# awslabs/flowgger

Measured on AMD Instinct MI355X. Metric: log lines/sec (RFC5424, 256B avg) at 1/2/4/8 MI355X; achieved HBM GB/s, higher is better.
Workload: dtype u8; 1 GPU; BASELINE configs[1]: RFC5424 no structured data, 100000000 lines/GPU @ 254 B avg (1000000-line tile x100 resident in HBM), 1% invalid lines; lines_per_gpu=100000000, bytes_per_gpu=25376525600, parallelism=lines sharded 1-way, no data-path collective, ok_lines_per_tile=990000

## Files before the change

flowgger_amd/csrc/fg_gelf.hip:

```cpp
#include "fg_fused.hpp"
#include "fg_numparse.hpp"
#include "fg_gelf2.hpp"

namespace fg {

using namespace gelf2;

enum : uint32_t { J_OK = 0, J_SYNTAX = 1, J_CTRL = 2 };
constexpr uint32_t V_NESTED = 6;
constexpr uint32_t kMaxDepth = 512;
constexpr uint32_t kMaxStored = 32;

struct Member {
    uint32_t key_b, key_e, key_esc;
    uint32_t kind;
    uint32_t v_b, v_e, v_esc;
    uint64_t bits;
    uint32_t end;
};

template <class R>
struct Gelf {
    R& rd;
    uint32_t len;
// ... 400 lines not shown
                    --j;
                }
                keypos[j] = pi;
            }
        }
        for (uint32_t i = 0; i < n; ++i) {
            Member m;
            g.member(keypos[i], &m);
            if (i + 1 < n) {
                uint32_t ne, nesc;
                g.scan_string(keypos[i + 1] + 1, &ne, &nesc);
                if (g.key_cmp(m.key_b, m.key_e, m.key_esc, keypos[i + 1] + 1, ne, nesc) == 0) continue;
            }
            uint32_t st = gelf_dispatch<EMIT>(g, m, r, t, slot, &cnt);
            if (st != G_OK) {
                r.status = st;
                return;
            }
        }
    } else {
        bool have_prev = false;
        Member prev;
        for (;;) {
            bool have_best = false;
            Member best;
            uint32_t p = g.skip_ws(0) + 1;
            for (uint32_t k = 0; k < n; ++k) {
                p = g.skip_ws(p);
                if (k) p = g.skip_ws(p + 1);
                Member m;
                g.member(p, &m);
                p = m.end;
                if (have_prev && g.key_cmp(m.key_b, m.key_e, m.key_esc, prev.key_b, prev.key_e, prev.key_esc) <= 0) continue;
                if (!have_best || g.key_cmp(m.key_b, m.key_e, m.key_esc, best.key_b, best.key_e, best.key_esc) <= 0) {
                    best = m;
                    have_best = true;
                }
            }
            if (!have_best) break;
            uint32_t st = gelf_dispatch<EMIT>(g, best, r, t, slot, &cnt);
            if (st != G_OK) {
                r.status = st;
                return;
            }
            prev = best;
            have_prev = true;
        }
    }
    if (!EMIT) r.n_ent = cnt;
}

template <class R>
__device__ __forceinline__ void gelf_line(R& rd, uint32_t len, uint32_t* keypos, uint32_t* stack, GRow& r, const DevTables& t) {
    Gelf<R> g{rd, len, false, stack};
    bool is_object = false;
    uint32_t e = gelf_validate(g, keypos, r, &is_object);
    if (e == J_CTRL) {
        g.retry = true;
        r = GRow();
        e = gelf_validate(g, keypos, r, &is_object);
        if (e == J_OK) r.flags |= FG_F_GELF_RETRY;
    }
    if (e != J_OK) {
        r.status = G_JSON;
        return;
    }
    if (!is_object) {
        r.status = G_EMPTY;
        return;
    }
    gelf_sorted_dispatch<false>(g, keypos, r, t, 0);
    if (r.status != G_OK) return;
    if (!r.have_ts) r.flags |= FG_F_TS_NOW;
    if (!r.have_host) r.status = G_NOHOST;
}

constexpr uint32_t kGelfLines = 64;
constexpr uint32_t kPending = 0xFCu;

inline uint32_t gelf_extra_lds(uint32_t tile, uint32_t lines) { return gelf2::extra_bytes(tile, lines); }

struct GelfFormat {
    static constexpr uint32_t kClasses = gelf2::kClasses;
    static __device__ __forceinline__ void classify_store(const uint4& q, uint16_t* bm16, uint32_t chunk, uint32_t stride, uint32_t term4) {
        uint32_t m[gelf2::kClasses + 1];
        gelf2::classify(q.x, q.y, q.z, q.w, m, term4);
        gelf2::store_classes(m, bm16, chunk, stride);
    }
    uint8_t* extra;
    uint32_t tile_cap, lines;
    unsigned long long* pacc;

    __device__ __forceinline__ RowOut decode(const GroupCtx& c, const DevTables& t) const {
        const uint32_t lane = threadIdx.x;
        const uint32_t len = (uint32_t)(c.o1 - c.o0);
        const bool in_tile = (c.o1 - c.a0) <= (uint64_t)c.span;
        const uint32_t base = (uint32_t)(c.o0 - c.a0);
        gelf2::Lds L = gelf2::carve(c.smem, c.bm16, tile_cap, extra, lines);
        L.ent_state = c.ent_state;
        L.alloc_chunk = t.alloc_chunk;
        const bool tile_lane = c.valid && in_tile && lane < lines && !(c.ablate & 4u);
        const gelf2::LineOut f = c.phase ? gelf2::decode_tile<true>(L, c.span, tile_lane, base, len, t, pacc)
                                         : gelf2::decode_tile<false>(L, c.span, tile_lane, base, len, t);
        RowOut o;
        const fg_span none{0, FG_NONE};
        const bool ok = f.handled && f.status == G_OK;
        o.meta = f.handled ? (f.status | (0xFFu << 8) | ((ok ? f.severity : 0xFFu) << 16) | ((ok ? f.flags : 0u) << 24)) : kPending;
        if (t.pending && c.valid && !f.handled) gstore(t.pending, 0, t.epoch);
        o.ts = (ok && f.have_ts) ? f.ts : 0.0;
        o.span[S_HOST] = ok ? fg_span{f.host_off, f.host_len} : none;
        o.span[S_APP] = none;
        o.span[S_PROC] = none;
        o.span[S_MSGID] = none;
        o.span[S_MSG] = ok ? fg_span{f.msg_off, f.msg_len} : none;
        o.span[S_FULL] = ok ? fg_span{f.full_off, f.full_len} : none;
        o.first = f.handled ? f.first : 0u;
        o.count = f.handled ? f.n_ent : 0u;
        return o;
    }
};

template <int NB, bool PROF, int MINW = 4, uint32_t TILE = 0, uint32_t LINES = 0>
__global__ __launch_bounds__(kWave, MINW) void k_gelf(const uint8_t* __restrict__ bytes, const uint64_t* __restrict__ offsets,
                                                  uint64_t n, DevTables t, uint32_t tile_cap_, uint32_t L_, uint64_t groups,
                                                  unsigned long long* prof, uint64_t* stash_base, FrameArgs fr) {
    const uint32_t tile_cap = TILE ? TILE : tile_cap_, L = LINES ? LINES : L_;
    extern __shared__ __attribute__((aligned(16))) uint8_t smem[];
    __shared__ unsigned long long pacc[PROF ? 10 : 1];
    GelfFormat fmt{smem + tile_cap + 64u + (tile_cap / 16u + 16u) * 2u * GelfFormat::kClasses, tile_cap, L, pacc};
    if (PROF && threadIdx.x < 10) pacc[threadIdx.x] = 0ull;
    {
        const gelf2::Lds lds = gelf2::carve(smem, reinterpret_cast<uint16_t*>(smem + tile_cap + 64u), tile_cap, fmt.extra, L);
        gelf2::init_lds(lds);
        gelf2::clear_dirty(lds, tile_cap);
    }
    __shared__ DevTables t_lds;
    if (threadIdx.x == 0) t_lds = t;
    __syncthreads();
    persistent_loop<NB, PROF>(bytes, offsets, n, t_lds, tile_cap, L, groups, prof, stash_base, fmt, fr);
    if (PROF) {
        __syncthreads();
        if (threadIdx.x < 10) atomicAdd(&prof[6 + threadIdx.x], pacc[threadIdx.x]);
    }
}

template <int NB, int MINW = 4, uint32_t TILE = 0, uint32_t LINES = 0>
__global__ __launch_bounds__(kWave, MINW) void k_gelf_fused(const uint8_t* __restrict__ bytes, DevTables t, uint32_t tile_cap_, uint32_t L_,
                                                         FusedArgs fa, uint32_t strip) {
    const uint32_t tile_cap = TILE ? TILE : tile_cap_, L = LINES ? LINES : L_;
    extern __shared__ __attribute__((aligned(16))) uint8_t smem[];
    GelfFormat fmt{smem + tile_cap + 64u + (tile_cap / 16u + 16u) * 2u * GelfFormat::kClasses, tile_cap, L, nullptr};
    {
        const gelf2::Lds lds = gelf2::carve(smem, reinterpret_cast<uint16_t*>(smem + tile_cap + 64u), tile_cap, fmt.extra, L);
        gelf2::init_lds(lds);
        gelf2::clear_dirty(lds, tile_cap);
    }
    __shared__ DevTables t_lds;
    __shared__ FusedArgs fa_lds;
    if (threadIdx.x == 0) {
        t_lds = t;
        fa_lds = fa;
    }
    __syncthreads();
    fused_loop<NB>(bytes, t_lds, tile_cap, L, fmt, fa_lds, strip, nullptr);
}

// ... 205 lines not shown
```

flowgger_amd/csrc/fg_pipeline.hpp:

```cpp
#pragma once
#include "fg_device.hpp"
#include "fg_plan_policy.hpp"
#include "fg_sparse_need.hpp"
#include "fg_wave.hpp"

namespace fg {

using u32x4 = unsigned int __attribute__((ext_vector_type(4)));

__device__ __forceinline__ uint32_t eq_flags(uint32_t x, uint32_t pat) {
    uint32_t s = ((x & 0x7F7F7F7Fu) ^ pat) + 0x7F7F7F7Fu;
    return ~(s | x) & 0x80808080u;
}
__device__ __forceinline__ uint32_t range_flags(uint32_t x) {
    uint32_t l = x & 0x7F7F7F7Fu;
    uint32_t ge33 = l + 0x5F5F5F5Fu;
    uint32_t le126 = l + 0x01010101u;
    return ge33 & ~le126 & ~x & 0x80808080u;
}
__device__ __forceinline__ uint32_t ctrl_flags(uint32_t x) {
    uint32_t ge32 = (x & 0x7F7F7F7Fu) + 0x60606060u;
    return ~(ge32 | x) & 0x80808080u;
}
__device__ __forceinline__ uint32_t gather16(uint32_t f0, uint32_t f1, uint32_t f2, uint32_t f3) {
// ... 149 lines not shown
    uint32_t span;
    bool valid;
    uint64_t li;
    uint64_t* stash;
    uint32_t ablate;
    uint32_t* ent_state;
    unsigned long long* phase;
    uint32_t tbase = 0;
    uint32_t tlen = 0;
    uint32_t last2 = 0;
    uint32_t tile_cap = 0;
};

template <uint32_t WORDS, class Unpack>
__device__ __forceinline__ bool stash_to_table(const GroupCtx& c, const DevTables& t, const EntAlloc& a, uint32_t n_ent, bool mine,
                                               Unpack un) {
    const uint32_t lane = threadIdx.x;
    const uint32_t cap = (c.span / 18u) & ~3u;
    if (a.total == 0u || a.total > cap || a.s.overflow || c.stash == nullptr || __any(n_ent != 0u && !mine)) return false;
    uint64_t* s_name = reinterpret_cast<uint64_t*>(const_cast<uint8_t*>(c.smem));
    uint64_t* s_val = s_name + cap;
    uint16_t* s_tf = reinterpret_cast<uint16_t*>(s_val + cap);
    __syncthreads();
    for (uint32_t k0 = 0; k0 < n_ent; k0 += 4u) {
        uint64_t w0[4], w1[4];
#pragma unroll
        for (uint32_t j = 0; j < 4u; ++j) {
            const uint32_t k = k0 + j < n_ent ? k0 + j : n_ent - 1u;
            w0[j] = c.stash[(k * WORDS) * kWave + lane];
            w1[j] = WORDS > 1u ? c.stash[(k * WORDS + 1u) * kWave + lane] : 0ull;
        }
#pragma unroll
        for (uint32_t j = 0; j < 4u; ++j) {
            if (k0 + j < n_ent) {
                uint64_t name, val;
                uint32_t tf;
                un(w0[j], w1[j], &name, &val, &tf);
                const uint32_t idx = a.ex + k0 + j;
                s_name[idx] = name;
                s_val[idx] = val;
                s_tf[idx] = (uint16_t)tf;
            }
        }
    }
    __syncthreads();
    for (uint32_t idx = lane; idx < a.total; idx += kWave) {
        const uint32_t slot = a.s.at(idx);
        const uint64_t name = s_name[idx];
        const uint32_t tf = s_tf[idx];
        t.ent_name[slot] = fg_span{(uint32_t)name, (uint32_t)(name >> 32)};
        t.ent_val[slot] = s_val[idx];
        t.ent_type[slot] = (uint8_t)(tf & 0xFFu);
        t.ent_flags[slot] = (uint8_t)(tf >> 8);
    }
    return true;
}


struct FrameArgs {
    uint32_t strip;
    const uint8_t* line_bad;
    uint32_t* ticket = nullptr;
    uint32_t ticket_base = 0;
    uint32_t taper0 = kNoTaper, taper1 = kNoTaper, taper2 = kNoTaper;
};

#define FG_STREAM_AUX 2
__device__ __forceinline__ uint4 stream_load(const uint4* p) {
    typedef uint32_t nt4 __attribute__((ext_vector_type(4)));
    const nt4 v = __builtin_nontemporal_load(reinterpret_cast<const nt4*>(p));
    return make_uint4(v.x, v.y, v.z, v.w);
}

template <class F, class = void>
struct tail_batch { static constexpr int value = 4; };
template <class F>
struct tail_batch<F, decltype((void)F::kTailBatch)> { static constexpr int value = F::kTailBatch; };

template <class F, class = void>
struct defer_row_store { static constexpr bool value = true; };
template <class F>
struct defer_row_store<F, decltype((void)F::kDeferRowStore)> { static constexpr bool value = F::kDeferRowStore; };

constexpr uint32_t kHeadCap = 1024;
template <class F, class = void>
struct head_cap { static constexpr uint32_t value = kHeadCap; };
template <class F>
struct head_cap<F, decltype((void)F::kHeadBytes)> { static constexpr uint32_t value = F::kHeadBytes; };

constexpr uint32_t kSparseHandful = 4;

template <int NB, bool PROF, class F, bool HEAD = false, uint32_t SPARSE = 0>
__device__ __forceinline__ void persistent_loop(const uint8_t* __restrict__ bytes, const uint64_t* __restrict__ offsets,
                                                uint64_t n, const DevTables& t, uint32_t tile_cap, uint32_t L, uint64_t chunk_lines,
                                                unsigned long long* prof, uint64_t* stash_base, F& fmt, FrameArgs fr) {
    static_assert(!HEAD || F::kClasses <= 1, "HEAD staging classifies one stage-A byte class at most");
    static_assert(SPARSE == 0 || (!HEAD && F::kClasses == 0), "the sparse window builds its need bitmap where a stage-A class bitmap would lie");
    static_assert(SPARSE % 16u == 0 && SPARSE <= 112u, "a line's run of chunks (at most (H + 4 + 14) / 16 + 1) must fit two bitmap words at any shift");
    const uint64_t kChunkLines = chunk_lines;
    extern __shared__ __attribute__((aligned(16))) uint8_t smem[];
    uint16_t* bm16 = reinterpret_cast<uint16_t*>(smem + tile_cap + 64u);
    const uint32_t bm_stride = tile_cap / 16u + 16u;
    uint4* dst = reinterpret_cast<uint4*>(smem);
    const uint32_t lane = threadIdx.x;
    const uint64_t G = gridDim.x;
    uint64_t* stash = stash_base ? stash_base + (uint64_t)blockIdx.x * (kStashEntries * kStashWords * kWave) : nullptr;

    const bool dyn = fr.ticket != nullptr;
    uint32_t tk_raw = 0;
    bool tk_pending = false;
    auto draw_ticket = [&]() {
        if (lane == 0u) tk_raw = __hip_atomic_fetch_add(fr.ticket, 1u, __ATOMIC_RELAXED, __HIP_MEMORY_SCOPE_AGENT);
        tk_pending = true;
    };
    uint64_t chunk = blockIdx.x;
    uint64_t p, hi_line;
    chunk_range(chunk, kChunkLines, fr.taper0, fr.taper1, fr.taper2, n, &p, &hi_line);
    if (dyn && p < n) draw_ticket();

    auto load_offsets = [&](uint64_t q, uint64_t* o0, uint64_t* o1) {
        const uint64_t li = q + lane;
        const bool in = lane < L && li < hi_line;
        *o0 = offsets[in ? li : hi_line];
        *o1 = offsets[in ? li + 1 : hi_line];
    };
    auto geometry = [&](uint64_t q, uint64_t o0, uint64_t o1, uint32_t* nl, uint64_t* a0, uint32_t* span) {
        const uint64_t left = hi_line - q;
        const uint32_t avail = left < (uint64_t)L ? (uint32_t)left : L;
        const uint32_t lo_l = (uint32_t)__builtin_amdgcn_readfirstlane((int)(uint32_t)o0);
        const uint32_t lo_h = (uint32_t)__builtin_amdgcn_readfirstlane((int)(uint32_t)(o0 >> 32));
        const uint64_t lo = (uint64_t)lo_l | ((uint64_t)lo_h << 32);
        *a0 = lo & ~15ull;
        const unsigned long long fit = __ballot(lane < avail && (o1 - *a0) <= (uint64_t)tile_cap);
        uint32_t cnt = fit == ~0ull ? 64u : (uint32_t)__builtin_ctzll(~fit);
        if (cnt == 0u) cnt = 1u;
        *nl = cnt;
        const uint32_t last = cnt - 1u;
        const uint32_t hi_l = (uint32_t)__builtin_amdgcn_readlane((int)(uint32_t)o1, (int)last);
        const uint32_t hi_h = (uint32_t)__builtin_amdgcn_readlane((int)(uint32_t)(o1 >> 32), (int)last);
        const uint64_t hi = (uint64_t)hi_l | ((uint64_t)hi_h << 32);
        const uint64_t want = hi - *a0;
        *span = want > tile_cap ? tile_cap : (uint32_t)((want + 15ull) & ~15ull);
    };
    auto load_window = [&](uint64_t a0, uint32_t span, u32x4* v) {
        __amdgpu_buffer_rsrc_t rsrc =
            __builtin_amdgcn_make_buffer_rsrc(const_cast<uint8_t*>(bytes + a0), (short)0, (int)span, 0x00020000);
#pragma unroll
        for (int k = 0; k < NB; ++k) v[k] = __builtin_amdgcn_raw_buffer_load_b128(rsrc, (int)(lane * 16u + k * 1024u), 0, FG_STREAM_AUX);
    };
    const uint32_t sparse_tail = fr.strip != FG_FRAME_NONE ? kSparseTailFramed : kSparseTailPlain;
    auto sparse_offsets = [&](uint64_t a0_, uint32_t span_, uint32_t nl_, uint64_t lo0, uint64_t lo1, bool dense, uint32_t* vo) {
        uint32_t* skip = reinterpret_cast<uint32_t*>(bm16);
        const uint32_t nchunk_ = span_ >> 4;
        const uint32_t nwin = nchunk_ < (uint32_t)NB * kWave ? nchunk_ : (uint32_t)NB * kWave;
        const uint32_t nword = 2u * NB + 2u < tile_cap / 32u + 8u ? 2u * NB + 2u : tile_cap / 32u + 8u;
        if (lane < nword) {
            const uint32_t c = lane * 32u;
            skip[lane] = !dense || c >= nchunk_ ? ~0u : nchunk_ - c >= 32u ? 0u : ~0u << (nchunk_ - c);
        }
        __syncthreads();
        if (!dense) {
            auto mark = [&](const NeedRange& r, bool on) {
                const bool go = on && r.n != 0u && r.c0 < nwin;
                const uint64_t m = go ? ((1ull << r.n) - 1ull) << (r.c0 & 31u) : 0ull;
                const uint32_t w = go ? r.c0 >> 5 : 0u;
                __hip_atomic_fetch_and(skip + w, ~(uint32_t)m, __ATOMIC_RELAXED, __HIP_MEMORY_SCOPE_WORKGROUP);
                __hip_atomic_fetch_and(skip + w + 1u, ~(uint32_t)(m >> 32), __ATOMIC_RELAXED, __HIP_MEMORY_SCOPE_WORKGROUP);
            };
            const uint32_t t0 = (uint32_t)lo0 - (uint32_t)a0_, t1 = (uint32_t)lo1 - (uint32_t)a0_;
            mark(need_head(t0, t1 - t0, SPARSE, sparse_tail, lane == 0u), lane < nl_);
            if (lane + 1u == nl_) mark(need_tail(t1, sparse_tail), true);
            __syncthreads();
        }
        const uint32_t half = lane >> 5, bit = lane & 31u, off = lane * 16u;
#pragma unroll
        for (int k = 0; k < NB; ++k) vo[k] = ((skip[2 * k + (int)half] >> bit) << 31) | off;
    };
    auto load_window_sparse = [&](uint64_t a0_, uint32_t span_, const uint32_t* vo, u32x4* v) {
        __amdgpu_buffer_rsrc_t rsrc =
            __builtin_amdgcn_make_buffer_rsrc(const_cast<uint8_t*>(bytes + a0_), (short)0, (int)span_, 0x00020000);
#pragma unroll
        for (int k = 0; k < NB; ++k) v[k] = __builtin_amdgcn_raw_buffer_load_b128(rsrc, (int)vo[k], k * 1024, FG_STREAM_AUX);
    };
    auto geometry_head = [&](uint64_t q, uint64_t o0, uint64_t o1, uint32_t* nl, uint32_t* span, uint32_t* st_out, uint32_t* tb_out) {
        const uint64_t left = hi_line - q;
        const uint32_t avail = left < (uint64_t)L ? (uint32_t)left : L;
        const uint64_t want = (o1 - o0) + (o0 & 15ull);
        uint32_t st = want >= head_cap<F>::value ? head_cap<F>::value : (uint32_t)((want + 15ull) & ~15ull);
        if (lane >= avail) st = 0u;
        uint32_t total;
        const uint32_t tb = wv::excl_sum(st, &total);
        const unsigned long long fit = __ballot(lane < avail && tb + st <= tile_cap);
        uint32_t cnt = fit == ~0ull ? 64u : (uint32_t)__builtin_ctzll(~fit);
        if (cnt == 0u) cnt = 1u;
        *nl = cnt;
        const uint32_t last = cnt - 1u;
        *span = (uint32_t)__builtin_amdgcn_readlane((int)tb, (int)last) + (uint32_t)__builtin_amdgcn_readlane((int)st, (int)last);
        *st_out = lane < cnt ? st : 0u;
        *tb_out = tb;
    };
    auto load_window_head = [&](uint64_t o0, uint32_t st, u32x4* v) {
#pragma unroll
        for (int k = 0; k < NB; ++k) {
            const uint32_t lo = (uint32_t)__builtin_amdgcn_readlane((int)(uint32_t)o0, k);
            const uint32_t hi = (uint32_t)__builtin_amdgcn_readlane((int)(uint32_t)(o0 >> 32), k);
            const uint32_t sk = (uint32_t)__builtin_amdgcn_readlane((int)st, k);
            const uint64_t b = ((uint64_t)lo | ((uint64_t)hi << 32)) & ~15ull;
            __amdgpu_buffer_rsrc_t rsrc = __builtin_amdgcn_make_buffer_rsrc(const_cast<uint8_t*>(bytes + b), (short)0, (int)sk, 0x00020000);
            v[k] = __builtin_amdgcn_raw_buffer_load_b128(rsrc, (int)(lane * 16u), 0, FG_STREAM_AUX);
        }
    };
    auto load_last2 = [&](uint64_t o0, uint64_t o1) -> uint32_t {
        const uint64_t len = o1 - o0;
        uint32_t r = 0;
        if (len >= 1u) r = bytes[o1 - 1u];
        if (len >= 2u) r |= (uint32_t)bytes[o1 - 2u] << 8;
        return r;
    };

    uint32_t* ent_state = reinterpret_cast<uint32_t*>(smem + tile_cap + 56u);
    if (lane < 2u) ent_state[lane] = 0u;
    if (p >= hi_line) return;
    uint64_t o0, o1, a0 = 0;
    uint32_t span, nl, st = 0, tb = 0, last2 = 0;
    load_offsets(p, &o0, &o1);
    u32x4 v[NB];
    if constexpr (HEAD) {
        geometry_head(p, o0, o1, &nl, &span, &st, &tb);
        load_window_head(o0, st, v);
        last2 = load_last2(o0, o1);
    } else if constexpr (SPARSE != 0) {
        geometry(p, o0, o1, &nl, &a0, &span);
        uint32_t vo[NB];
        sparse_offsets(a0, span, nl, o0, o1, false, vo);
        load_window_sparse(a0, span, vo, v);
    } else {
        geometry(p, o0, o1, &nl, &a0, &span);
        load_window(a0, span, v);
    }
    bool dense = false, dense_next = false, dense_then = false;
    RowOut pend{};
    uint64_t pend_li = 0;
    bool pend_valid = false;
    uint64_t acc0 = 0, acc1 = 0, acc2 = 0, acc3 = 0, iters = 0, tm0 = 0, tm1 = 0, tm2 = 0, tm3 = 0;
    const uint32_t ablate = PROF ? (uint32_t)prof[5] : 0u;
    const uint32_t term4 = fr.strip == FG_FRAME_LINE ? 0x0A0A0A0Au : fr.strip == FG_FRAME_NUL ? 0u : wv::kNoTerm;

    for (;;) {
        uint64_t pn = p + nl;
        if (pn >= hi_line) {
            if (dyn) {
                if (!tk_pending) draw_ticket();
                const uint32_t tk = (uint32_t)__builtin_amdgcn_readfirstlane((int)tk_raw);
                chunk = (uint64_t)(uint32_t)(tk - fr.ticket_base) + G;
                tk_pending = false;
                chunk_range(chunk, kChunkLines, fr.taper0, fr.taper1, fr.taper2, n, &pn, &hi_line);
                if (pn < n) draw_ticket();
            } else {
                chunk += G;
                chunk_range(chunk, kChunkLines, kNoTaper, kNoTaper, kNoTaper, n, &pn, &hi_line);
            }
        }
        const bool more = pn < n;
        uint64_t no0 = 0, no1 = 0;
        if (more) load_offsets(pn, &no0, &no1);
        if (PROF) {
            tm0 = __builtin_amdgcn_s_memtime();
            __builtin_amdgcn_s_waitcnt(0x0F70);
            tm1 = __builtin_amdgcn_s_memtime();
        }
        FG_MARK(A);
        const uint32_t nchunk = span >> 4;
        const uint32_t nrow = HEAD ? nl : (nchunk + kWave - 1u) / kWave;
        if constexpr (HEAD) {
#pragma unroll
            for (int k = 0; k < NB; ++k) {
                if ((uint32_t)k < nl) {
                    const uint32_t tk = (uint32_t)__builtin_amdgcn_readlane((int)tb, k), sk = (uint32_t)__builtin_amdgcn_readlane((int)st, k);
                    if (lane * 16u < sk) {
                        const uint4 q = make_uint4(v[k][0], v[k][1], v[k][2], v[k][3]);
                        dst[(tk >> 4) + lane] = q;
                        if constexpr (F::kClasses != 0) F::classify_store(q, bm16, (tk >> 4) + lane, bm_stride, term4);
                    }
                }
            }
            constexpr uint32_t HB = tail_batch<F>::value >= 8 ? 8u : 4u;
            for (uint32_t r0 = NB; r0 < nl; r0 += HB) {
                uint4 w[HB];
                uint32_t tk[HB], sk[HB];
#pragma unroll
                for (uint32_t j = 0; j < HB; ++j) {
                    const uint32_t r = r0 + j < nl ? r0 + j : nl - 1u;
                    const uint32_t lo = (uint32_t)__builtin_amdgcn_readlane((int)(uint32_t)o0, (int)r);
                    const uint32_t hi = (uint32_t)__builtin_amdgcn_readlane((int)(uint32_t)(o0 >> 32), (int)r);
                    tk[j] = (uint32_t)__builtin_amdgcn_readlane((int)tb, (int)r);
                    sk[j] = (uint32_t)__builtin_amdgcn_readlane((int)st, (int)r);
                    const uint64_t b = ((uint64_t)lo | ((uint64_t)hi << 32)) & ~15ull;
                    __amdgpu_buffer_rsrc_t rsrc = __builtin_amdgcn_make_buffer_rsrc(const_cast<uint8_t*>(bytes + b), (short)0, (int)sk[j], 0x00020000);
                    const u32x4 x = __builtin_amdgcn_raw_buffer_load_b128(rsrc, (int)(lane * 16u), 0, FG_STREAM_AUX);
                    w[j] = make_uint4(x[0], x[1], x[2], x[3]);
                }
#pragma unroll
                for (uint32_t j = 0; j < HB; ++j)
                    if (lane * 16u < sk[j]) {
                        dst[(tk[j] >> 4) + lane] = w[j];
                        if constexpr (F::kClasses != 0) F::classify_store(w[j], bm16, (tk[j] >> 4) + lane, bm_stride, term4);
                    }
            }
        } else {
#pragma unroll
        for (int k = 0; k < NB; ++k) {
            if ((uint32_t)k < nrow) {
                uint32_t idx = k * kWave + lane;
                uint4 q = make_uint4(v[k][0], v[k][1], v[k][2], v[k][3]);
                dst[idx] = q;
                F::classify_store(q, bm16, idx, bm_stride, idx < nchunk ? term4 : wv::kPastSpan);
            }
        }
        }
        if (!HEAD && nrow > (uint32_t)NB) {
            const uint4* __restrict__ src = reinterpret_cast<const uint4*>(bytes + a0);
            const uint32_t last = nchunk - 1u;
            constexpr int TB = tail_batch<F>::value;
            for (uint32_t c0 = NB * kWave; c0 < nchunk; c0 += kWave * TB) {
                uint4 w[TB];
#pragma unroll
                for (int k = 0; k < TB; ++k) {
                    const uint32_t idx = c0 + k * kWave + lane;
                    w[k] = stream_load(src + (idx < last ? idx : last));
                }
#pragma unroll
                for (int k = 0; k < TB; ++k) {
                    if (k == 0 || c0 + k * kWave < nchunk) {
                        const uint32_t idx = c0 + k * kWave + lane, ci = idx < last ? idx : last;
                        dst[ci] = w[k];
                        F::classify_store(w[k], bm16, ci, bm_stride, term4);
                    }
                }
            }
            if constexpr (SPARSE != 0) __builtin_amdgcn_s_waitcnt(0x0F70);
        }
        __builtin_amdgcn_sched_barrier(0);
        FG_MARK(S);
        if (PROF) {
            __builtin_amdgcn_s_waitcnt(0xC07F);
            tm2 = __builtin_amdgcn_s_memtime();
        }
        uint64_t pa0 = 0;
        uint32_t pspan = 0, pnl = 0, pst = 0, ptb = 0, plast2 = 0;
        if (more) {
            if constexpr (HEAD) geometry_head(pn, no0, no1, &pnl, &pspan, &pst, &ptb);
            else geometry(pn, no0, no1, &pnl, &pa0, &pspan);
        }
        uint32_t pvo[SPARSE != 0 ? NB : 1];
        if constexpr (SPARSE != 0) {
            dense_next = dense_then;
            if (more) sparse_offsets(pa0, pspan, pnl, no0, no1, dense_next, pvo);
        }
        FG_MARK(ST);
        if (pend_valid && !(ablate & 1u)) store_row(t, pend_li, pend);
        FG_MARK(W0);
        if (more) {
            if constexpr (HEAD) {
                load_window_head(no0, pst, v);
                plast2 = load_last2(no0, no1);
            } else if constexpr (SPARSE != 0) {
                load_window_sparse(pa0, pspan, pvo, v);
            } else {
                load_window(pa0, pspan, v);
            }
        }
        __builtin_amdgcn_sched_barrier(0);
        FG_MARK(W1);
        FG_MARK(B);
        if (PROF) tm3 = __builtin_amdgcn_s_memtime();
        __syncthreads();
        if (!(ablate & 2u)) {
            const uint64_t li = p + lane;
            const bool valid = lane < nl;
            uint64_t e1 = o1;
            uint32_t l2 = last2;
            if (fr.strip != FG_FRAME_NONE) {
                uint32_t b1 = last2 & 0xFFu, b2 = (last2 >> 8) & 0xFFu;
                if constexpr (!HEAD) {
                    const uint64_t len = o1 - o0;
                    const bool over = nl == 1u && __builtin_amdgcn_readfirstlane((int)((o1 - a0) > (uint64_t)span)) != 0;
                    if (over) {
                        FG_RARE_BEGIN();
                        if (valid && len >= 1u) b1 = bytes[o1 - 1u];
                        if (valid && len >= 2u) b2 = bytes[o1 - 2u];
                        FG_RARE_END();
                    } else if (valid) {
                        const uint32_t q = (uint32_t)(o1 - a0);
                        if (len >= 1u) b1 = smem[q - 1u];
                        if (len >= 2u) b2 = smem[q - 2u];
                    }
                }
                if (valid && e1 > o0) {
                    if (fr.strip == FG_FRAME_LINE) {
                        if (b1 == '\n') {
                            --e1;
                            if (e1 > o0 && b2 == '\r') --e1;
                        }
                    } else if (b1 == 0u) {
                        --e1;
                    }
                    if (HEAD && e1 != o1) {
                        l2 = 0u;
                        if (e1 - o0 >= 1u) l2 = bytes[e1 - 1];
                        if (e1 - o0 >= 2u) l2 |= (uint32_t)bytes[e1 - 2] << 8;
                    }
                }
            }
            GroupCtx c{bytes, smem, bm16, o0, e1, a0, span, valid, li, (ablate & 8u) ? nullptr : stash, ablate, ent_state, PROF ? prof + 6 : nullptr};
            c.tile_cap = tile_cap;
            if constexpr (HEAD) {
                const uint32_t al = (uint32_t)(o0 & 15ull), len = (uint32_t)(e1 - o0);
                c.tbase = tb + al;
                c.tlen = st == 0u ? 0u : (st - al < len ? st - al : len);
                c.last2 = l2;
            }
            if constexpr (SPARSE != 0) {
                const uint32_t len = (uint32_t)(e1 - o0);
                c.tbase = (uint32_t)(o0 - a0);
                c.tlen = dense || len < SPARSE ? len : SPARSE;
                c.last2 = 0u;
                if (valid && e1 > o0 && (o1 - a0) <= (uint64_t)span) {
                    const uint32_t q = (uint32_t)(e1 - a0);
                    c.last2 = smem[q - 1u];
                    if (len >= 2u) c.last2 |= (uint32_t)smem[q - 2u] << 8;
                }
            }
            pend = fmt.decode(c, t);
            if constexpr (SPARSE != 0) {
                const uint32_t nh = (uint32_t)__popcll(__ballot(valid && pend.handed));
                dense_then = dense ? nh != 0u : nh > kSparseHandful;
            }
            if (fr.line_bad && valid && fr.line_bad[li]) {
                pend.meta = FG_ST_BAD_UTF8 | (0xFFu << 8) | (0xFFu << 16);
                pend.ts = 0.0;
#pragma unroll
                for (int k = 0; k < 6; ++k) pend.span[k] = fg_span{0, FG_NONE};
                pend.count = 0;
            }
            pend_li = li;
            pend_valid = valid;
            if (!defer_row_store<F>::value) {
                if (pend_valid && !(ablate & 1u)) store_row(t, pend_li, pend);
                pend_valid = false;
            }
        }
        if (PROF) {
            __builtin_amdgcn_sched_barrier(0);
            __builtin_amdgcn_s_waitcnt(0xC07F);
            uint64_t tm4 = __builtin_amdgcn_s_memtime();
            acc0 += tm1 - tm0;
            acc1 += tm2 - tm1;
            acc2 += tm3 - tm2;
            acc3 += tm4 - tm3;
            iters += 1;
        }
        FG_MARK(Z);
        if (!more) break;
        __syncthreads();
        p = pn;
        nl = pnl;
        o0 = no0;
        o1 = no1;
        a0 = pa0;
        span = pspan;
        if constexpr (SPARSE != 0) dense = dense_next;
        if constexpr (HEAD) {
            st = pst;
            tb = ptb;
            last2 = plast2;
        }
    }
    if (pend_valid && !(ablate & 1u)) store_row(t, pend_li, pend);
    if (PROF && lane == 0) {
        atomicAdd(&prof[0], (unsigned long long)acc0);
        atomicAdd(&prof[1], (unsigned long long)acc1);
        atomicAdd(&prof[2], (unsigned long long)acc2);
        atomicAdd(&prof[3], (unsigned long long)acc3);
        atomicAdd(&prof[4], (unsigned long long)iters);
    }
}

}

#include <cstdio>
#include <cstdlib>

#include "fg_cus.hpp"

namespace fg {
constexpr int kComputeBoundWindow = 2;

inline void take_tickets(FrameArgs* fr, TicketSlot* tk, const LaunchPlan& p) {
    if (!tk || !tk->d_word || !tk->h_val || p.chunks + p.blocks >= 0xFFFFFFFFull || p.blocks > p.chunks) return;
    if (!p.tickets) return;
    fr->ticket = tk->d_word;
    fr->ticket_base = *tk->h_val;
    fr->taper0 = p.taper[0], fr->taper1 = p.taper[1], fr->taper2 = p.taper[2];
    *tk->h_val += (uint32_t)p.chunks;
}

template <class K>
inline int plan_launch(K kernel, uint64_t n, uint64_t avg_len, uint32_t extra_lds, uint32_t max_tile, uint32_t stash_blocks, LaunchPlan* p,
                       const fg_launch_opts& lo, const PlanFormat& pf = PlanFormat()) {
    static_cast<LaunchGeometry&>(*p) = launch_geometry(n, avg_len, extra_lds, max_tile, lo, pf);
    const int cus = device_cus();
    if (cus < 1) return -1;
    int per_cu = 0;
    if (hipOccupancyMaxActiveBlocksPerMultiprocessor(&per_cu, kernel, kWave, p->lds) != hipSuccess || per_cu < 1) per_cu = 1;
    if (lo.waves_per_cu > 0 && per_cu > (int)lo.waves_per_cu) per_cu = (int)lo.waves_per_cu;
    uint64_t blocks = (uint64_t)per_cu * (uint64_t)cus;
    if (blocks > p->groups) blocks = p->groups;
    if (stash_blocks && blocks > stash_blocks) blocks = stash_blocks;
    const ChunkPlan cp = plan_chunks(n, blocks, p->L, p->g, p->full, pf.ticket_from, lo, pf.taper);
    p->chunk = cp.chunk;
    p->chunks = cp.chunks;
    p->tickets = cp.tickets;
    for (int j = 0; j < 3; ++j) p->taper[j] = cp.taper[j];
    p->blocks = cp.blocks;
    return 0;
}

#if defined(FG_PROF_BUILD)
inline bool prof_requested() { return getenv("FG_PROF") != nullptr; }
#define FG_PROF_TWIN(...) (__VA_ARGS__)
#else
constexpr bool prof_requested() { return false; }
#define FG_PROF_TWIN(...) nullptr
#endif
struct ProfRun {
    unsigned long long* d = nullptr;
    unsigned long long h[16] = {0, 0, 0, 0, 0, 0, 0, 0, 0, 0, 0, 0, 0, 0, 0, 0};
    bool begin(hipStream_t stream) {
#if defined(FG_PROF_BUILD)
        if (const char* e = getenv("FG_ABLATE")) h[5] = (unsigned long long)atoi(e);
#endif
        if (hipMalloc((void**)&d, sizeof(h)) != hipSuccess) return false;
        (void)hipMemcpyAsync(d, h, sizeof(h), hipMemcpyHostToDevice, stream);
        return true;
    }
    void end(hipStream_t stream, const char* name, const LaunchPlan& p) {
        (void)hipStreamSynchronize(stream);
        (void)hipMemcpy(h, d, sizeof(h), hipMemcpyDeviceToHost);
        (void)hipFree(d);
        const double it = h[4] ? (double)h[4] : 1.0;
        fprintf(stderr,
// ... 55 lines not shown
```

flowgger_amd/csrc/fg_rfc5424.hip:

```cpp
#include <cstdio>
#include <cstdlib>

#include "fg_fused.hpp"
#include "fg_sd2.hpp"
#include "fg_tsfast.hpp"

namespace fg {

enum : uint32_t {
    E_OK = 0,
    E_BOM = 1,
    E_BRACKETS = 2,
    E_INVPRI = 3,
    E_NOVER = 4,
    E_BADVER = 5,
    E_NOTS = 6,
    E_BADTS = 7,
    E_NOHOST = 8,
    E_NOAPP = 9,
    E_NOPROC = 10,
    E_NOMSGID = 11,
    E_NODATA = 12,
    E_NOMSG = 13,
    E_MALFORMED = 14,
// ... 826 lines not shown
                sd_walk<true>(rd, r.data0, len, &msg_at, &cnt, t, first);
            } else {
                FG_RARE_BEGIN();
                GlobalReader rd(reinterpret_cast<const uint32_t*>(bytes), o0);
                sd_walk<true>(rd, r.data0, len, &msg_at, &cnt, t, first);
                FG_RARE_END();
            }
        }
    }

    tick(8);
    RowOut o;
    const bool ok = r.status == E_OK;
    o.meta = r.status | (r.facility << 8) | (r.severity << 16) | (r.flags << 24);
    o.ts = ok ? r.ts : 0.0;
#pragma unroll
    for (int k = 0; k < 6; ++k) o.span[k] = ok ? fg_span{r.off[k], r.len[k]} : fg_span{0, FG_NONE};
    o.first = first;
    o.count = r.n_ent;
    if constexpr (kSparse) {
        o.handed = valid && in_window && (coop ||
                             (len > HB && ((route & (R_GENERIC | R_TAIL)) != 0u || ((route & R_TRIM) != 0u && !trim_settled) || f.d0 + 3u > HB)));
    }
    if constexpr (HEAD) {
        unsigned long long todo = __ballot(coop);
        while (todo) {
            const int src = (int)__builtin_ctzll(todo);
            todo &= todo - 1ull;
            auto rl64 = [&](uint64_t x) -> uint64_t {
                return (uint64_t)(uint32_t)__builtin_amdgcn_readlane((int)(uint32_t)x, src) |
                       ((uint64_t)(uint32_t)__builtin_amdgcn_readlane((int)(uint32_t)(x >> 32), src) << 32);
            };
            const uint64_t ro0 = rl64(o0), ro1 = rl64(o1), rli = rl64(c.li);
            const uint64_t ra0 = ro0 & ~15ull;
            const uint32_t rspan = (uint32_t)((ro1 - ra0 + 15ull) & ~15ull);
            __syncthreads();
            {
                __amdgpu_buffer_rsrc_t rsrc = __builtin_amdgcn_make_buffer_rsrc(const_cast<uint8_t*>(bytes + ra0), (short)0, (int)rspan, 0x00020000);
                uint4* dst = reinterpret_cast<uint4*>(const_cast<uint8_t*>(smem));
                const uint32_t nrow = (rspan + 1023u) >> 10;
                for (uint32_t r0 = 0; r0 < nrow; r0 += 4u) {
                    u32x4 w[4];
#pragma unroll
                    for (uint32_t j = 0; j < 4u; ++j) w[j] = __builtin_amdgcn_raw_buffer_load_b128(rsrc, (int)(lane * 16u + (r0 + j) * 1024u), 0, FG_STREAM_AUX);
#pragma unroll
                    for (uint32_t j = 0; j < 4u; ++j)
                        if (r0 + j < nrow) dst[(r0 + j) * kWave + lane] = make_uint4(w[j][0], w[j][1], w[j][2], w[j][3]);
                }
            }
            __syncthreads();
            GroupCtx c2{bytes, smem, bm16, ro0, ro1, ra0, rspan, lane == 0u, rli, c.stash, ablate, c.ent_state, nullptr};
            c2.tile_cap = c.tile_cap;
            Rfc5424FormatT<false, SDX, false, 0, true> whole;
            const RowOut w = whole.decode(c2, t);
            auto b32 = [&](uint32_t x) -> uint32_t { return (uint32_t)__builtin_amdgcn_readfirstlane((int)x); };
            const uint32_t g_meta = b32(w.meta), g_first = b32(w.first), g_count = b32(w.count);
            const uint64_t tsb = (uint64_t)__builtin_bit_cast(unsigned long long, w.ts);
            const uint32_t g_ts0 = b32((uint32_t)tsb), g_ts1 = b32((uint32_t)(tsb >> 32));
            uint32_t g_off[6], g_len[6];
#pragma unroll
            for (int k = 0; k < 6; ++k) {
                g_off[k] = b32(w.span[k].off);
                g_len[k] = b32(w.span[k].len);
            }
            if ((int)lane == src) {
                o.meta = g_meta;
                o.ts = __builtin_bit_cast(double, (unsigned long long)((uint64_t)g_ts0 | ((uint64_t)g_ts1 << 32)));
#pragma unroll
                for (int k = 0; k < 6; ++k) o.span[k] = fg_span{g_off[k], g_len[k]};
                o.first = g_first;
                o.count = g_count;
            }
        }
    }
    tick(9);
    if (PROF && pacc && lane == 0)
        for (int k = 0; k < 10; ++k) pacc[k] += (unsigned long long)pc[k];
    return o;
    }
};

using Rfc5424Format = Rfc5424FormatT<false>;

template <int NB, bool PROF, bool HEAD = false, bool SDX = false>
__global__ __launch_bounds__(kWave, 2) void k_rfc5424(const uint8_t* __restrict__ bytes,
                                                     const uint64_t* __restrict__ offsets, uint64_t n, DevTables t,
                                                     uint32_t tile_cap, uint32_t L, uint64_t groups,
                                                     unsigned long long* prof, uint64_t* stash_base, FrameArgs fr) {
    Rfc5424FormatT<HEAD, SDX, PROF> fmt;
    if constexpr (PROF) {
        __shared__ unsigned long long pacc[10];
        if (threadIdx.x < 10) pacc[threadIdx.x] = 0ull;
        fmt.pacc = pacc;
        __syncthreads();
        persistent_loop<NB, PROF, Rfc5424FormatT<HEAD, SDX, PROF>, HEAD>(bytes, offsets, n, t, tile_cap, L, groups, prof, stash_base, fmt, fr);
        __syncthreads();
        if (prof && threadIdx.x < 10) atomicAdd(&prof[6 + threadIdx.x], pacc[threadIdx.x]);
    } else if constexpr (SDX) {
        __shared__ DevTables t_lds;
        if (threadIdx.x == 0) t_lds = t;
        __syncthreads();
        persistent_loop<NB, PROF, Rfc5424FormatT<HEAD, SDX, PROF>, HEAD>(bytes, offsets, n, t_lds, tile_cap, L, groups, prof, stash_base, fmt, fr);
    } else {
        persistent_loop<NB, PROF, Rfc5424FormatT<HEAD, SDX, PROF>, HEAD>(bytes, offsets, n, t, tile_cap, L, groups, prof, stash_base, fmt, fr);
    }
}

template <int NB, bool PROF, uint32_t H>
__global__ __launch_bounds__(kWave, 2) void k_rfc5424_sparse(const uint8_t* __restrict__ bytes, const uint64_t* __restrict__ offsets, uint64_t n,
                                                            DevTables t, uint32_t tile_cap, uint32_t L, uint64_t groups,
                                                            unsigned long long* prof, uint64_t* stash_base, FrameArgs fr) {
    Rfc5424FormatT<true, false, PROF, H> fmt;
    if constexpr (PROF) {
        __shared__ unsigned long long pacc[10];
        if (threadIdx.x < 10) pacc[threadIdx.x] = 0ull;
        fmt.pacc = pacc;
        __syncthreads();
        persistent_loop<NB, PROF, Rfc5424FormatT<true, false, PROF, H>, false, H>(bytes, offsets, n, t, tile_cap, L, groups, prof, stash_base, fmt, fr);
        __syncthreads();
        if (prof && threadIdx.x < 10) atomicAdd(&prof[6 + threadIdx.x], pacc[threadIdx.x]);
    } else {
        persistent_loop<NB, PROF, Rfc5424FormatT<true, false, PROF, H>, false, H>(bytes, offsets, n, t, tile_cap, L, groups, prof, stash_base, fmt, fr);
    }
}

template <int NB, bool SDX>
__global__ __launch_bounds__(kWave, 2) void k_rfc5424_fused(const uint8_t* __restrict__ bytes, DevTables t, uint32_t tile_cap, uint32_t L,
                                                           uint64_t* stash_base, FusedArgs fa, uint32_t strip) {
    Rfc5424FormatT<false, SDX, false> fmt;
    __shared__ DevTables t_lds;
    __shared__ FusedArgs fa_lds;
    if (threadIdx.x == 0) {
        t_lds = t;
        fa_lds = fa;
    }
    __syncthreads();
    fused_loop<NB>(bytes, t_lds, tile_cap, L, fmt, fa_lds, strip, stash_base);
}

}

extern "C" uint64_t fg_stash_bytes(uint32_t blocks) {
    return (uint64_t)blocks * fg::kStashEntries * fg::kStashWords * fg::kWave * sizeof(uint64_t);
}

namespace {
template <bool HEAD, bool SDX>
auto rfc5424_kernels(const char* name) {
    return fg::kernels(fg::k_rfc5424<fg::kWindowKiB, false, HEAD, SDX>, FG_PROF_TWIN(fg::k_rfc5424<fg::kWindowKiB, true, HEAD, SDX>), name);
}
}

extern "C" int fg_launch_rfc5424(const uint8_t* d_bytes, const uint64_t* d_offsets, uint64_t n, const fg::DevTables* t,
                                 uint64_t avg_len, hipStream_t stream, uint64_t* stash, uint32_t stash_blocks, uint32_t strip,
                                 const uint8_t* line_bad, const fg_launch_opts* lo, fg::TicketSlot* tk) {
    if (n == 0) return 0;
    const fg::Variant v = fg::pick_variant(avg_len, lo->flags);
    const bool sparse = fg::pick_sparse(avg_len, lo->flags, v);
    const auto ks = sparse ? fg::kernels(fg::k_rfc5424_sparse<fg::kWindowKiB, false, fg::kSparseHead>,
                                         FG_PROF_TWIN(fg::k_rfc5424_sparse<fg::kWindowKiB, true, fg::kSparseHead>), "rfc5424 (sparse)")
                    : v.pairs ? (v.head ? rfc5424_kernels<true, true>("rfc5424 (head, pairs)") : rfc5424_kernels<false, true>("rfc5424 (pairs)"))
                            : (v.head ? rfc5424_kernels<true, false>("rfc5424 (head)") : rfc5424_kernels<false, false>("rfc5424"));
    const fg::PlanFormat pf = v.pairs ? fg::PlanFormat().classes(2u).lds_tile(fg::sd2::extra_bytes).tile(12288u).chunk(128u).tickets_from(4u)
                              : v.head ? fg::PlanFormat()
                                       : fg::rfc5424_walk_format(avg_len);
    const uint32_t max_tile = v.pairs ? 36864u : fg::kMaxTile;
    const uint64_t plan_len = v.head ? (avg_len < fg::kHeadCap ? avg_len : fg::kHeadCap) : avg_len;
    const uint32_t sb = stash ? stash_blocks : 0u;
    if (stash_blocks == 0) stash = nullptr;
    return fg::plan_and_launch(ks, fg::DecodeCall{n, t, stream, fg::FrameArgs{strip, line_bad}, lo, tk}, plan_len, 0u, max_tile, sb, pf,
                               [&](auto k, const fg::LaunchPlan& p, const fg::DevTables& tt, const fg::FrameArgs& fr, unsigned long long* prof) {
                                   hipLaunchKernelGGL(k, dim3(p.blocks), dim3(fg::kWave), p.lds, stream, d_bytes, d_offsets, n, tt, p.tile, p.L, p.chunk,
                                                      prof, stash, fr);
                               });
}

extern "C" int fg_launch_rfc5424_fused(const uint8_t* d_bytes, uint64_t nbytes, const fg::DevTables* t, const fg::FusedGeom* g, hipStream_t stream,
                                       uint64_t* stash, uint32_t stash_blocks, uint32_t strip, int final_, uint64_t* d_offsets, uint64_t cap,
                                       uint8_t* scratch, const fg_launch_opts* lo, unsigned long long** d_total) {
    const bool sdx = g->variant == 1u;
    const auto kernel = sdx ? fg::k_rfc5424_fused<12, true> : fg::k_rfc5424_fused<16, false>;
    const uint32_t base_lds = fg::tile_lds(g->tile, sdx ? 2u : 1u) + (sdx ? fg::sd2::extra_bytes(g->tile) : 0u);
    if (stash_blocks == 0) stash = nullptr;
    return fg::launch_fused(kernel, fg::FusedCall{nbytes, t, g, stream, strip, final_, d_offsets, cap, scratch, lo, d_total}, base_lds, stash ? stash_blocks : 0u,
                            [&](auto k, uint32_t blocks, uint32_t lds, const fg::DevTables& tt, const fg::FusedArgs& fa) {
                                hipLaunchKernelGGL(k, dim3(blocks), dim3(fg::kWave), lds, stream, d_bytes, tt, g->tile, g->L, stash, fa, strip);
                            });
}
// ... 1 lines not shown
```

Before: 18.21 billion lines/s.

## Prefetch line offsets two groups ahead and cap VGPRs for the RFC5424 kernel

The persistent loop now computes the next-next group and loads its line offsets one iteration earlier, so the offset load latency overlaps a full group of decode work instead of being exposed before the window geometry step. GELF opts out via a trait. The non-profiled NB=20 RFC5424 kernel is also specialized with an explicit VGPR cap of 104, and the ticket atomic address is laundered through an opaque zero. The extra prefetch adds live registers, which the VGPR cap may turn into spills.

```diff
diff --git a/flowgger_amd/csrc/fg_gelf.hip b/flowgger_amd/csrc/fg_gelf.hip
--- a/flowgger_amd/csrc/fg_gelf.hip
+++ b/flowgger_amd/csrc/fg_gelf.hip
@@ -506,6 +506,7 @@
 
 struct GelfFormat {
     static constexpr uint32_t kClasses = gelf2::kClasses;
+    static constexpr bool kOffsetsAhead = false;
     static __device__ __forceinline__ void classify_store(const uint4& q, uint16_t* bm16, uint32_t chunk, uint32_t stride, uint32_t term4) {
         uint32_t m[gelf2::kClasses + 1];
         gelf2::classify(q.x, q.y, q.z, q.w, m, term4);
diff --git a/flowgger_amd/csrc/fg_pipeline.hpp b/flowgger_amd/csrc/fg_pipeline.hpp
--- a/flowgger_amd/csrc/fg_pipeline.hpp
+++ b/flowgger_amd/csrc/fg_pipeline.hpp
@@ -255,6 +255,11 @@
 template <class F>
 struct defer_row_store<F, decltype((void)F::kDeferRowStore)> { static constexpr bool value = F::kDeferRowStore; };
 
+template <class F, class = void>
+struct offsets_ahead { static constexpr bool value = true; };
+template <class F>
+struct offsets_ahead<F, decltype((void)F::kOffsetsAhead)> { static constexpr bool value = F::kOffsetsAhead; };
+
 constexpr uint32_t kHeadCap = 1024;
 template <class F, class = void>
 struct head_cap { static constexpr uint32_t value = kHeadCap; };
@@ -283,21 +288,39 @@
     uint32_t tk_raw = 0;
     bool tk_pending = false;
     auto draw_ticket = [&]() {
-        if (lane == 0u) tk_raw = __hip_atomic_fetch_add(fr.ticket, 1u, __ATOMIC_RELAXED, __HIP_MEMORY_SCOPE_AGENT);
+        uint32_t zero = 0;
+        asm volatile("" : "+v"(zero));
+        if (lane == 0u) tk_raw = __hip_atomic_fetch_add(fr.ticket + zero, 1u, __ATOMIC_RELAXED, __HIP_MEMORY_SCOPE_AGENT);
         tk_pending = true;
     };
     uint64_t chunk = blockIdx.x;
-    uint64_t p, hi_line;
-    chunk_range(chunk, kChunkLines, fr.taper0, fr.taper1, fr.taper2, n, &p, &hi_line);
+    uint64_t p, hi_n;
+    chunk_range(chunk, kChunkLines, fr.taper0, fr.taper1, fr.taper2, n, &p, &hi_n);
     if (dyn && p < n) draw_ticket();
 
-    auto load_offsets = [&](uint64_t q, uint64_t* o0, uint64_t* o1) {
+    auto next_group = [&](uint64_t q, uint64_t* hi) -> uint64_t {
+        if (q >= *hi) {
+            if (dyn) {
+                if (!tk_pending) draw_ticket();
+                const uint32_t tk = (uint32_t)__builtin_amdgcn_readfirstlane((int)tk_raw);
+                chunk = (uint64_t)(uint32_t)(tk - fr.ticket_base) + G;
+                tk_pending = false;
+                chunk_range(chunk, kChunkLines, fr.taper0, fr.taper1, fr.taper2, n, &q, hi);
+                if (q < n) draw_ticket();
+            } else {
+                chunk += G;
+                chunk_range(chunk, kChunkLines, kNoTaper, kNoTaper, kNoTaper, n, &q, hi);
+            }
+        }
+        return q;
+    };
+    auto load_offsets = [&](uint64_t q, uint64_t hi, uint64_t* o0, uint64_t* o1) {
         const uint64_t li = q + lane;
-        const bool in = lane < L && li < hi_line;
-        *o0 = offsets[in ? li : hi_line];
-        *o1 = offsets[in ? li + 1 : hi_line];
-    };
-    auto geometry = [&](uint64_t q, uint64_t o0, uint64_t o1, uint32_t* nl, uint64_t* a0, uint32_t* span) {
+        const bool in = lane < L && li < hi;
+        *o0 = offsets[in ? li : hi];
+        *o1 = offsets[in ? li + 1 : hi];
+    };
+    auto geometry = [&](uint64_t q, uint64_t hi_line, uint64_t o0, uint64_t o1, uint32_t* nl, uint64_t* a0, uint32_t* span) {
         const uint64_t left = hi_line - q;
         const uint32_t avail = left < (uint64_t)L ? (uint32_t)left : L;
         const uint32_t lo_l = (uint32_t)__builtin_amdgcn_readfirstlane((int)(uint32_t)o0);
@@ -355,7 +378,7 @@
 #pragma unroll
         for (int k = 0; k < NB; ++k) v[k] = __builtin_amdgcn_raw_buffer_load_b128(rsrc, (int)vo[k], k * 1024, FG_STREAM_AUX);
     };
-    auto geometry_head = [&](uint64_t q, uint64_t o0, uint64_t o1, uint32_t* nl, uint32_t* span, uint32_t* st_out, uint32_t* tb_out) {
+    auto geometry_head = [&](uint64_t q, uint64_t hi_line, uint64_t o0, uint64_t o1, uint32_t* nl, uint32_t* span, uint32_t* st_out, uint32_t* tb_out) {
         const uint64_t left = hi_line - q;
         const uint32_t avail = left < (uint64_t)L ? (uint32_t)left : L;
         const uint64_t want = (o1 - o0) + (o0 & 15ull);
@@ -393,22 +416,27 @@
 
     uint32_t* ent_state = reinterpret_cast<uint32_t*>(smem + tile_cap + 56u);
     if (lane < 2u) ent_state[lane] = 0u;
-    if (p >= hi_line) return;
+    if (p >= hi_n) return;
     uint64_t o0, o1, a0 = 0;
     uint32_t span, nl, st = 0, tb = 0, last2 = 0;
-    load_offsets(p, &o0, &o1);
+    load_offsets(p, hi_n, &o0, &o1);
+    if constexpr (HEAD) geometry_head(p, hi_n, o0, o1, &nl, &span, &st, &tb);
+    else geometry(p, hi_n, o0, o1, &nl, &a0, &span);
+    constexpr bool kAhead = offsets_ahead<F>::value;
+    uint64_t pn = p, no0 = 0, no1 = 0;
+    if constexpr (kAhead) {
+        pn = next_group(p + nl, &hi_n);
+        load_offsets(pn, hi_n, &no0, &no1);
+    }
     u32x4 v[NB];
     if constexpr (HEAD) {
-        geometry_head(p, o0, o1, &nl, &span, &st, &tb);
         load_window_head(o0, st, v);
         last2 = load_last2(o0, o1);
     } else if constexpr (SPARSE != 0) {
-        geometry(p, o0, o1, &nl, &a0, &span);
         uint32_t vo[NB];
         sparse_offsets(a0, span, nl, o0, o1, false, vo);
         load_window_sparse(a0, span, vo, v);
     } else {
-        geometry(p, o0, o1, &nl, &a0, &span);
         load_window(a0, span, v);
     }
     bool dense = false, dense_next = false, dense_then = false;
@@ -420,23 +448,11 @@
     const uint32_t term4 = fr.strip == FG_FRAME_LINE ? 0x0A0A0A0Au : fr.strip == FG_FRAME_NUL ? 0u : wv::kNoTerm;
 
     for (;;) {
-        uint64_t pn = p + nl;
-        if (pn >= hi_line) {
-            if (dyn) {
-                if (!tk_pending) draw_ticket();
-                const uint32_t tk = (uint32_t)__builtin_amdgcn_readfirstlane((int)tk_raw);
-                chunk = (uint64_t)(uint32_t)(tk - fr.ticket_base) + G;
-                tk_pending = false;
-                chunk_range(chunk, kChunkLines, fr.taper0, fr.taper1, fr.taper2, n, &pn, &hi_line);
-                if (pn < n) draw_ticket();
-            } else {
-                chunk += G;
-                chunk_range(chunk, kChunkLines, kNoTaper, kNoTaper, kNoTaper, n, &pn, &hi_line);
-            }
-        }
+        if constexpr (!kAhead) pn = next_group(p + nl, &hi_n);
         const bool more = pn < n;
-        uint64_t no0 = 0, no1 = 0;
-        if (more) load_offsets(pn, &no0, &no1);
+        if constexpr (!kAhead) {
+            if (more) load_offsets(pn, hi_n, &no0, &no1);
+        }
         if (PROF) {
             tm0 = __builtin_amdgcn_s_memtime();
             __builtin_amdgcn_s_waitcnt(0x0F70);
@@ -522,8 +538,13 @@
         uint64_t pa0 = 0;
         uint32_t pspan = 0, pnl = 0, pst = 0, ptb = 0, plast2 = 0;
         if (more) {
-            if constexpr (HEAD) geometry_head(pn, no0, no1, &pnl, &pspan, &pst, &ptb);
-            else geometry(pn, no0, no1, &pnl, &pa0, &pspan);
+            if constexpr (HEAD) geometry_head(pn, hi_n, no0, no1, &pnl, &pspan, &pst, &ptb);
+            else geometry(pn, hi_n, no0, no1, &pnl, &pa0, &pspan);
+        }
+        uint64_t hi_nn = hi_n, pnn = pn, nno0 = 0, nno1 = 0;
+        if constexpr (kAhead) {
+            if (more) pnn = next_group(pn + pnl, &hi_nn);
+            load_offsets(pnn, hi_nn, &nno0, &nno1);
         }
         uint32_t pvo[SPARSE != 0 ? NB : 1];
         if constexpr (SPARSE != 0) {
@@ -640,6 +661,12 @@
         nl = pnl;
         o0 = no0;
         o1 = no1;
+        if constexpr (kAhead) {
+            pn = pnn;
+            hi_n = hi_nn;
+            no0 = nno0;
+            no1 = nno1;
+        }
         a0 = pa0;
         span = pspan;
         if constexpr (SPARSE != 0) dense = dense_next;
diff --git a/flowgger_amd/csrc/fg_rfc5424.hip b/flowgger_amd/csrc/fg_rfc5424.hip
--- a/flowgger_amd/csrc/fg_rfc5424.hip
+++ b/flowgger_amd/csrc/fg_rfc5424.hip
@@ -932,11 +932,10 @@
 
 using Rfc5424Format = Rfc5424FormatT<false>;
 
-template <int NB, bool PROF, bool HEAD = false, bool SDX = false>
-__global__ __launch_bounds__(kWave, 2) void k_rfc5424(const uint8_t* __restrict__ bytes,
-                                                     const uint64_t* __restrict__ offsets, uint64_t n, DevTables t,
-                                                     uint32_t tile_cap, uint32_t L, uint64_t groups,
-                                                     unsigned long long* prof, uint64_t* stash_base, FrameArgs fr) {
+template <int NB, bool PROF, bool HEAD, bool SDX>
+__device__ __forceinline__ void rfc5424_kernel_body(const uint8_t* __restrict__ bytes, const uint64_t* __restrict__ offsets, uint64_t n,
+                                                    const DevTables& t, uint32_t tile_cap, uint32_t L, uint64_t groups,
+                                                    unsigned long long* prof, uint64_t* stash_base, const FrameArgs& fr) {
     Rfc5424FormatT<HEAD, SDX, PROF> fmt;
     if constexpr (PROF) {
         __shared__ unsigned long long pacc[10];
@@ -954,6 +953,19 @@
     } else {
         persistent_loop<NB, PROF, Rfc5424FormatT<HEAD, SDX, PROF>, HEAD>(bytes, offsets, n, t, tile_cap, L, groups, prof, stash_base, fmt, fr);
     }
+}
+template <int NB, bool PROF, bool HEAD = false, bool SDX = false>
+__global__ __launch_bounds__(kWave, 2) void k_rfc5424(const uint8_t* __restrict__ bytes,
+                                                     const uint64_t* __restrict__ offsets, uint64_t n, DevTables t,
+                                                     uint32_t tile_cap, uint32_t L, uint64_t groups,
+                                                     unsigned long long* prof, uint64_t* stash_base, FrameArgs fr) {
+    rfc5424_kernel_body<NB, PROF, HEAD, SDX>(bytes, offsets, n, t, tile_cap, L, groups, prof, stash_base, fr);
+}
+template <>
+__global__ __launch_bounds__(kWave, 2) __attribute__((amdgpu_num_vgpr(104))) void k_rfc5424<20, false, false, false>(
+    const uint8_t* __restrict__ bytes, const uint64_t* __restrict__ offsets, uint64_t n, DevTables t, uint32_t tile_cap, uint32_t L,
+    uint64_t groups, unsigned long long* prof, uint64_t* stash_base, FrameArgs fr) {
+    rfc5424_kernel_body<20, false, false, false>(bytes, offsets, n, t, tile_cap, L, groups, prof, stash_base, fr);
 }
 
 template <int NB, bool PROF, uint32_t H>
```

Measured after the change: 18.47 billion lines/s (median of 6 runs). 1.4% higher.
